# zfkuang/PaletteNeRF

Hardware: AMD Instinct MI355X
Metric: rendered_samples_per_sec (higher is better)
Workload: dtype f32 (field: f16x3 split products, fp32 accumulate); 1 GPU; configs[1]: NeRF-synthetic lego geometry (scene S0), -m nerf inference, 800x800, 1 view(s)/step, camera moving (one pose of the path per step); march_mode=native, fused_field=True, field_precision=f16x3, half_tables=False, ray_order=tile8, frames_in_flight=1, gathered_floats_per_ray=0, rccl_ranks=1, parallelism=single GPU

## Files before the change

palettenerf_amd/csrc/frame.hip:

```cpp
#include "pnr_common.hpp"
#include "march_core.hpp"
#include "grid_core.hpp"
#include "field_core.hpp"
#include "frame_plan.hpp"
#include <hip/hip_ext.h>
#include <vector>
#include <stdlib.h>

uint64_t pnr_internal_edit_device_bytes();
int pnr_internal_edit_upload(const pnr_palette_edit* edit, void* dst, hipStream_t s);
int pnr_internal_palette_field_forward(const pnr_palette_field_args* a, pnr_stream_t stream, int waves12);

namespace pnr {

struct FrameCtl {
    int32_t n_alive, n_step, step, done;
    int32_t iterations, pad0;
    unsigned long long rendered;
    unsigned long long rows;
    int32_t pad1[6];
};
static_assert(sizeof(FrameCtl) == 64, "FrameCtl layout");

constexpr uint32_t kHdr = 4;
// ... 113 lines not shown
        if (fin.depth_raw) fin.depth_raw[r] = d;
        depth[r] = (fin.on & 2) ? finish_depth(fin, d, r) : d;
    }
    if (q < 3) { const float v = simage[(size_t)i * 3 + q]; image[(size_t)r * 3 + q] = (fin.on & 1) ? finish_channel(fin, v, sws[i], r, q) : v; }
    if (saux) {
        if (q * 4 < aux_stride) {
            float4 v = *reinterpret_cast<const float4*>(saux + (size_t)i * aux_stride + q * 4);
            if (q == 0 && (fin.on & 4)) {
                const float w = sws[i];
                v.x = finish_channel(fin, v.x, w, r, 0); v.y = finish_channel(fin, v.y, w, r, 1); v.z = finish_channel(fin, v.z, w, r, 2);
            }
            *reinterpret_cast<float4*>(aux + (size_t)r * aux_stride + q * 4) = v;
        }
    } else if (aux && (fin.on & 4) && q < 3) {
        aux[(size_t)r * aux_stride + q] = finish_channel(fin, aux[(size_t)r * aux_stride + q], sws[i], r, q);
    }
}

#ifdef PNR_MARCH_STATS
__device__ unsigned long long g_march_stats[8];
__device__ unsigned int g_march_max[64];
__device__ unsigned int g_march_hist[2][32];
__device__ unsigned int g_march_kinds[64][8];
#endif
__device__ __forceinline__ uint32_t shfl_xor_fresh(uint32_t v, int off) {
    int lane = (int)__builtin_amdgcn_mbcnt_hi(~0u, __builtin_amdgcn_mbcnt_lo(~0u, 0u));
    asm volatile("" : "+v"(lane));
    return (uint32_t)__builtin_amdgcn_ds_bpermute((lane ^ off) << 2, (int)v);
}
__device__ __forceinline__ unsigned long long shfl_xor_fresh(unsigned long long v, int off) {
    return ((unsigned long long)shfl_xor_fresh((uint32_t)(v >> 32), off) << 32) | shfl_xor_fresh((uint32_t)v, off);
}
__device__ __forceinline__ unsigned long long block_sum_u64(unsigned long long v, unsigned long long* sh ) {
    for (int off = PNR_WAVE / 2; off > 0; off >>= 1) v += shfl_xor_fresh(v, off);
    __syncthreads();
    if ((threadIdx.x & (PNR_WAVE - 1)) == 0) sh[threadIdx.x / PNR_WAVE] = v;
    __syncthreads();
    unsigned long long t = 0;
    for (int wv = 0; wv < (int)(kRayBlock / PNR_WAVE); wv++) t += sh[wv];
    return t;
}


#ifdef PNR_MARCH_TIMING
constexpr int kTimingWaves = 8192;
__device__ unsigned long long g_march_timing[kTimingWaves * 8];
__device__ int g_march_timing_iter = 3;
#define PNR_STAMP(k) do { if (timing && (threadIdx.x & 63) == 0) g_march_timing[(size_t)twave * 8 + (k)] = wall_clock64(); } while (0)
#else
#define PNR_STAMP(k) do { } while (0)
#endif
#ifndef PNR_MARCH_WAVES
#define PNR_MARCH_WAVES 4
#endif
#ifndef PNR_MARCH_WAVES_Q
#define PNR_MARCH_WAVES_Q 5
#endif
template <bool MIP, bool POW2, int MODE>
__global__ void __launch_bounds__(kRayBlock) __attribute__((amdgpu_waves_per_eu(MODE == 2 ? PNR_MARCH_WAVES_Q : PNR_MARCH_WAVES))) k_frame_march(const FrameCtl* __restrict__ prev, FrameCtl* __restrict__ cur, const int32_t* __restrict__ alive_prev,
                                                           int32_t* __restrict__ rays_alive, const int32_t* __restrict__ counts ,
                                                           int32_t* __restrict__ counts_cur ,
                                                           int32_t* __restrict__ scratch_rw, uint32_t N, uint32_t max_steps,
                                                           const int32_t* __restrict__ partials_prev, uint32_t n_partials_prev,
                                                           const float* __restrict__ rays_t, const float* __restrict__ rays_o,
                                                           const float* __restrict__ rays_d, MarchParams p, const uint8_t* __restrict__ grid,
                                                           const float* __restrict__ fars, float* __restrict__ xyzs, float* __restrict__ dirs,
                                                           float* __restrict__ deltas, const uint32_t* __restrict__ mip,
                                                           int32_t* __restrict__ emitted_partials , uint32_t budget,
                                                           int32_t* __restrict__ qctr_all , StragglerRec* __restrict__ qrecs,
                                                           uint8_t* __restrict__ rowflag ,
                                                           const float* __restrict__ noises ) {
    __shared__ int csum[kRayBlock / PNR_WAVE];
    __shared__ unsigned long long red[kRayBlock / PNR_WAVE];
    __shared__ CoopShared coop[MODE == 1 ? kRayBlock / PNR_WAVE : 1];
#ifdef PNR_MARCH_TIMING
    const bool timing = prev->iterations + 1 == g_march_timing_iter && blockIdx.x * (kRayBlock / PNR_WAVE) < (uint32_t)kTimingWaves;
    const uint32_t twave = blockIdx.x * (kRayBlock / PNR_WAVE) + threadIdx.x / PNR_WAVE;
#endif
    PNR_STAMP(0);
    constexpr int kCountLoads = 8, kMipLoads = 5;
    const uint32_t max_chunks = (N + kRayBlock - 1) / kRayBlock;
    int32_t cv[kCountLoads];
#pragma unroll
    for (int u = 0; u < kCountLoads; u++) {
        const uint32_t j = threadIdx.x + (uint32_t)u * kRayBlock;
        cv[u] = j < max_chunks ? counts[j] : 0;
    }
    const uint32_t slot0 = blockIdx.x * kRayBlock + threadIdx.x;
    int index0 = slot0 < N ? alive_prev[slot0] : -1;
    extern __shared__ uint32_t mip_smem[];
    const uint32_t mip_n = MIP ? 2 * p.mip_words + 8 : 0;
    const bool mip_fast = MIP && mip_n <= (uint32_t)kMipLoads * kRayBlock * 4 && (mip_n & 3u) == 0;
    if (mip_fast) {
#pragma unroll
        for (int u = 0; u < kMipLoads; u++) {
            const uint32_t i = (threadIdx.x + (uint32_t)u * kRayBlock) * 4;
            if (i < mip_n) __builtin_amdgcn_global_load_lds((const __attribute__((address_space(1))) void*)(&mip[i]),
                                                            (__attribute__((address_space(3))) void*)(&mip_smem[i]), 16, 0, 0);
        }
    }
    if (prev->done) { if (blockIdx.x == 0 && threadIdx.x == 0) *cur = *prev; asm volatile("s_waitcnt vmcnt(0)" ::: "memory"); return; }
    const uint32_t n_prev = (uint32_t)prev->n_alive, nchunks = (n_prev + kRayBlock - 1) / kRayBlock;
    if (blockIdx.x >= nchunks && blockIdx.x != 0) { if (threadIdx.x == 0) emitted_partials[blockIdx.x] = 0; asm volatile("s_waitcnt vmcnt(0)" ::: "memory"); return; }
    if (slot0 >= n_prev) index0 = -1;
    unsigned long long part = 0;
#pragma unroll
    for (int u = 0; u < kCountLoads; u++) {
        const uint32_t j = threadIdx.x + (uint32_t)u * kRayBlock;
        if (j >= nchunks) cv[u] = 0;
        part += ((unsigned long long)(uint32_t)cv[u] << 32) | (j < blockIdx.x ? (unsigned long long)(uint32_t)cv[u] : 0ull);
    }
    for (uint32_t j = threadIdx.x + kCountLoads * kRayBlock; j < nchunks; j += kRayBlock) {
        const unsigned long long v = (unsigned long long)(uint32_t)counts[j];
        part += (v << 32) | (j < blockIdx.x ? v : 0ull);
    }
    const unsigned long long sums = block_sum_u64(part, red);
    const uint32_t n_alive = (uint32_t)(sums >> 32);
    const uint32_t n_step = (uint32_t)schedule_n_step((int)N, (int)n_alive);
    const int step_now = prev->step + prev->n_step;
    const bool done = n_alive == 0 || (uint32_t)step_now >= max_steps;
    if (blockIdx.x == 0) {
        unsigned long long e = 0;
        for (uint32_t j = threadIdx.x; j < n_partials_prev; j += kRayBlock) e += (unsigned long long)partials_prev[j];
        const unsigned long long emitted_prev = block_sum_u64(e, red);
        if (threadIdx.x == 0) {
            FrameCtl c = *prev;
            c.rendered += emitted_prev;
            c.rows += (unsigned long long)n_prev * (unsigned long long)prev->n_step;
            c.step = step_now;
            c.iterations += 1;
            c.n_alive = (int32_t)n_alive;
            c.n_step = (int32_t)n_step;
            c.done = done;
            c.pad0 = scratch_rw[1];
            *cur = c;
            scratch_rw[2] = 0;
            qctr_all[((c.iterations + 1) & 1) * kQueueCtrs] = 0;
        }
    }
    if (done || blockIdx.x >= nchunks) { if (threadIdx.x == 0) emitted_partials[blockIdx.x] = 0; asm volatile("s_waitcnt vmcnt(0)" ::: "memory"); return; }
    const int lane = threadIdx.x & (PNR_WAVE - 1), wave = threadIdx.x / PNR_WAVE;
    PNR_STAMP(1);
    const uint32_t* mip_lds = nullptr;
    if (mip_fast) {
        asm volatile("s_waitcnt vmcnt(0)" ::: "memory");
        __syncthreads();
        mip_lds = mip_smem;
    } else {
        mip_lds = stage_mip(mip, MIP ? p.mip_words : 0);
    }
    PNR_STAMP(2);
    uint32_t emitted = 0;
    uint32_t base = (uint32_t)(sums & 0xffffffffull), summed_to = blockIdx.x;
    for (uint32_t chunk = blockIdx.x; chunk < nchunks; chunk += gridDim.x) {
        if (threadIdx.x == 0) counts_cur[chunk] = 0;
        int index = index0;
        if (chunk != blockIdx.x) {
            unsigned long long pre = 0;
            for (uint32_t j = summed_to + threadIdx.x; j < chunk; j += kRayBlock) pre += (unsigned long long)counts[j];
            base += (uint32_t)block_sum_u64(pre, red);
            summed_to = chunk;
            const uint32_t slot = chunk * kRayBlock + threadIdx.x;
            index = slot < n_prev ? alive_prev[slot] : -1;
        }
        const int keep = index >= 0 ? 1 : 0;
        const unsigned long long alive_mask = __ballot(keep);
        if (lane == 0) csum[wave] = __popcll(alive_mask);
        __syncthreads();
        int woff = 0;
        for (int wv = 0; wv < wave; wv++) woff += csum[wv];
        __syncthreads();
        PNR_STAMP(3);
        uint32_t n = 0, step = 0;
        float t = 0.0f, far = -FLT_MAX, last_t = 0.0f;
        RayCtx c = {};
        if (keep) {
            n = base + (uint32_t)woff + (uint32_t)__popcll(alive_mask & ((1ull << lane) - 1ull));
            rays_alive[n] = index;
            ctx_init(c, rays_o + (size_t)index * 3, rays_d + (size_t)index * 3, p, grid, mip_lds);
            t = rays_t[index];
            const BoxHit bh = clip_to_box(c, fars[index]);
            far = bh.far;
            const float noise = (noises && prev->iterations == -1) ? noises[index] : 0.0f;
            t = fmaf(clampf(t * c.dt_gamma, c.dt_min, c.dt_max), noise, t);
            last_t = t;
            t = skip_to_box<MIP && POW2>(c, bh, t);
        }
        PNR_STAMP(4);
#ifdef PNR_MARCH_TIMING
        uint32_t my_probes = 0;
#endif
#ifdef PNR_MARCH_STATS
        unsigned long long probes = 0, empties = 0;
        unsigned int kinds[8] = {0, 0, 0, 0, 0, 0, 0, 0};
#endif
        bool active = keep && t < far;
        [[maybe_unused]] bool queued = false;
        [[maybe_unused]] uint32_t step_queued = 0;
        for (uint32_t round = 0;; round++) {
            const unsigned long long am = __ballot(active);
            if (am == 0ull) break;
            if constexpr (MODE == 1) { if (p.coop && __popcll(am) <= kCoopRays) break; }
            if constexpr (MODE == 2) {
                const bool give_up = active && round - step >= budget;
                const unsigned long long gm = __ballot(give_up);
                if (gm != 0ull) {
                    int32_t* qctr = qctr_all + ((prev->iterations + 1) & 1) * kQueueCtrs;
                    const int leader = __ffsll((long long)gm) - 1;
                    int slot0 = 0;
                    if (lane == leader) slot0 = atomicAdd(&qctr[0], __popcll(gm));
                    slot0 = __builtin_amdgcn_readlane(slot0, leader);
                    if (give_up) {
                        StragglerRec r;
                        r.n = (int32_t)n; r.index = index; r.step = (int32_t)step; r.t = t; r.last_t = last_t; r.far = far; r.pad0 = 0; r.pad1 = 0;
                        qrecs[(uint32_t)slot0 + (uint32_t)__popcll(gm & ((1ull << lane) - 1ull))] = r;
                        queued = true; step_queued = step; active = false;
                    }
                    if (gm == am) break;
                }
            }
            if (active) {
                float x, y, z, dt;
#ifdef PNR_MARCH_TIMING
                my_probes++;
#endif
#ifdef PNR_MARCH_STATS
                probes++;
                int kind = 7;
                const bool hit = march_probe<MIP, POW2>(c, t, x, y, z, dt, &kind);
                kinds[kind & 7]++;
                if (!hit) empties++;
#else
                const bool hit = march_probe<MIP, POW2>(c, t, x, y, z, dt);
#endif
                if (hit) {
                    const size_t row = (size_t)n * n_step + step;
                    float* px = xyzs + row * 3;
                    float* pd = dirs + row * 3;
                    float* pl = deltas + row * 2;
                    px[0] = x; px[1] = y; px[2] = z;
                    pd[0] = c.dx; pd[1] = c.dy; pd[2] = c.dz;
                    t += dt;
                    pl[0] = dt; pl[1] = t - last_t;
                    last_t = t;
                    step++;
                }
                active = t < far && step < n_step;
            }
        }
        if constexpr (MODE == 1) {
            if (p.coop && __ballot(active) != 0ull)
                step = march_coop_tail<MIP, POW2>(coop[wave], p, grid, mip_lds, n_step, active, c, t, far, last_t, n, step, xyzs, dirs, deltas);
        }
#ifdef PNR_MARCH_STATS
        if (keep) {
            const int so = prev->iterations + 1 == 0 ? 0 : 4;
            if (atomicMax(&g_march_max[(prev->iterations + 1) & 63], (unsigned int)probes) < (unsigned int)probes)
                for (int kk = 0; kk < 8; kk++) g_march_kinds[(prev->iterations + 1) & 63][kk] = kinds[kk];
            atomicAdd(&g_march_stats[so + 0], probes); atomicAdd(&g_march_stats[so + 1], empties); atomicAdd(&g_march_stats[so + 3], 1ull);
            atomicAdd(&g_march_hist[so ? 1 : 0][probes > 31 ? 31 : (int)probes], 1u);
            for (int kk = 0; kk < 8; kk++) if (kinds[kk]) atomicAdd(&g_march_kinds[so ? 63 : 62][kk], kinds[kk]);
        }
        {
            unsigned long long mx = probes;
            for (int off = 32; off > 0; off >>= 1) { unsigned long long o = __shfl_xor(mx, off, 64); mx = o > mx ? o : mx; }
            if ((threadIdx.x & 63) == 0) atomicAdd(&g_march_stats[prev->iterations + 1 == 0 ? 2 : 6], mx);
        }
#endif
        if (keep) {
            emitted += step;
            if constexpr (MODE == 2) {
                uint8_t* pf = rowflag + (size_t)n * n_step;
                for (uint32_t k = 0; k < n_step; k++) pf[k] = (queued && k >= step_queued) ? 1 : 0;
                if (queued) step = n_step;
            }
            float* pl = deltas + ((size_t)n * n_step + step) * 2;
            for (; step < n_step; step++) { pl[0] = 0.0f; pl[1] = 0.0f; pl += 2; }
        }
        PNR_STAMP(5);
#ifdef PNR_MARCH_TIMING
        if (timing) {
            uint32_t mp = my_probes, ml = c.n_loads;
            for (int off = 32; off > 0; off >>= 1) { mp = max(mp, (uint32_t)__shfl_xor((int)mp, off, 64)); ml = max(ml, (uint32_t)__shfl_xor((int)ml, off, 64)); }
            const uint32_t crowd = (uint32_t)__popcll(__ballot(my_probes >= 5u));
            if ((threadIdx.x & 63) == 0) { g_march_timing[(size_t)twave * 8 + 6] = mp; g_march_timing[(size_t)twave * 8 + 7] = ml | ((unsigned long long)crowd << 16); }
        }
#endif
    }
    __shared__ uint32_t wsum[kRayBlock / PNR_WAVE];
    for (int off = PNR_WAVE / 2; off > 0; off >>= 1) emitted += shfl_xor_fresh(emitted, off);
    if ((threadIdx.x & (PNR_WAVE - 1)) == 0) wsum[threadIdx.x / PNR_WAVE] = emitted;
    __syncthreads();
    if (threadIdx.x == 0) {
        uint32_t tot = 0;
        for (int wv = 0; wv < (int)(kRayBlock / PNR_WAVE); wv++) tot += wsum[wv];
        emitted_partials[blockIdx.x] = (int32_t)tot;
    }
}

enum GridKind { GK_SINGLE = 0, GK_PAIR = 1, GK_TRIPLE = 2, GK_HALF1 = 3, GK_HALF2 = 4, GK_HALF3 = 5 };
struct GridArgs {
    const float* xyzs; const float* deltas;
    const void* table[3]; float* enc[3];
    const int32_t* offsets; LevelParams lp;
    uint32_t level_stride; float bound, two_bound, inv_two_bound ; uint32_t gridtype;
};
struct LevelCtx { uint32_t off0, hashmap_size, resolution; float scale; uint32_t kind; };
__device__ __forceinline__ LevelCtx level_ctx(const GridArgs& g, uint32_t level) {
    LevelCtx lc;
    lc.off0 = (uint32_t)g.offsets[level];
    lc.hashmap_size = (uint32_t)g.offsets[level + 1] - lc.off0;
    lc.scale = g.lp.scale[level];
    lc.resolution = g.lp.resolution[level];
    lc.kind = level_kind<3>(g.gridtype, lc.hashmap_size, lc.resolution);
    return lc;
}
template <uint32_t CMUL>
__device__ __forceinline__ bool grid_corner_rows(const GridArgs& g, const LevelCtx& lc, uint32_t b, uint32_t idxs[8], float pos[3]) {
    float xyz[3];
#pragma unroll
    for (int d = 0; d < 3; d++) xyz[d] = g.xyzs[(size_t)b * 3 + d];
    asm volatile("" : "+v"(xyz[0]), "+v"(xyz[1]), "+v"(xyz[2]));
    float in[3];
    if (!unit_cube_of(xyz, g.bound, g.two_bound, g.inv_two_bound, in)) return false;
    uint32_t pg[3];
    grid_cell<3>(in, lc.scale, false, pg, pos);
    corner_rows<3, CMUL>(lc.kind, g.gridtype, false, lc.hashmap_size, lc.resolution, pg, idxs);
    return true;
}
template <int KIND, bool ORDERED = true>
__device__ __forceinline__ void grid_row(const GridArgs& g, const LevelCtx& lc, uint32_t level, const void* __restrict__ table, float* __restrict__ enc0, uint32_t b) {
    uint32_t idxs[8];
    float pos[3];
    const size_t o = ((size_t)level * g.level_stride + b) * 2;
    if constexpr (KIND == GK_TRIPLE) {
        float4 out = make_float4(0.0f, 0.0f, 0.0f, 0.0f);
        float2 outc = make_float2(0.0f, 0.0f);
        if (grid_corner_rows<1>(g, lc, b, idxs, pos)) {
            f32x4 v[8];
            f32x2 vc[8];
            float ws[8];
            const f32x4* tab = static_cast<const f32x4*>(table) + (size_t)lc.off0 * 2;
#pragma unroll
            for (int i = 0; i < 8; i++) v[i] = tab[(size_t)idxs[i] * 2];
#pragma unroll
            for (int i = 0; i < 8; i++) vc[i] = reinterpret_cast<const f32x2*>(tab + 1)[(size_t)idxs[i] * 4];
            corner_weights<3>(pos, ws);
#pragma unroll
            for (uint32_t idx = 0; idx < 8; idx++) {
                out.x = fmaf(ws[idx], v[idx].x, out.x); out.y = fmaf(ws[idx], v[idx].y, out.y);
                out.z = fmaf(ws[idx], v[idx].z, out.z); out.w = fmaf(ws[idx], v[idx].w, out.w);
                outc.x = fmaf(ws[idx], vc[idx].x, outc.x); outc.y = fmaf(ws[idx], vc[idx].y, outc.y);
            }
        }
        *reinterpret_cast<float2*>(enc0 + o) = make_float2(out.x, out.y);
        *reinterpret_cast<float2*>(g.enc[1] + o) = make_float2(out.z, out.w);
        *reinterpret_cast<float2*>(g.enc[2] + o) = outc;
    } else {
        constexpr bool HALF = KIND == GK_HALF1 || KIND == GK_HALF2 || KIND == GK_HALF3;
        constexpr int NT = KIND == GK_HALF3 ? 3 : ((KIND == GK_HALF2 || KIND == GK_PAIR) ? 2 : 1);
        constexpr int NW = HALF ? (NT == 3 ? 4 : NT) : 2 * NT;
        typedef uint32_t RowT __attribute__((ext_vector_type(NW)));
        typedef typename std::conditional<HALF, __half, float>::type AccT;
        AccT out[HALF ? 2 * NW : NW];
#pragma unroll
        for (int ch = 0; ch < 2 * NT; ch++) out[ch] = AccT(0.0f);
        if (grid_corner_rows<1>(g, lc, b, idxs, pos)) cell_interp<RowT, HALF, ORDERED>(static_cast<const RowT*>(table) + lc.off0, idxs, pos, out);
        *reinterpret_cast<float2*>(enc0 + o) = make_float2(to_f32(out[0]), to_f32(out[1]));
        if constexpr (NT >= 2) *reinterpret_cast<float2*>(g.enc[1] + o) = make_float2(to_f32(out[2]), to_f32(out[3]));
        if constexpr (NT == 3) *reinterpret_cast<float2*>(g.enc[2] + o) = make_float2(to_f32(out[4]), to_f32(out[5]));
    }
}

__device__ __forceinline__ uint32_t dpp_swap_pair(uint32_t x) { return (uint32_t)__builtin_amdgcn_update_dpp(0, (int)x, 0xB1 , 0xF, 0xF, true); }
template <int KIND>
__device__ __forceinline__ void grid_pair_level(const GridArgs& g, const LevelCtx& lc, uint32_t level, const void* __restrict__ table, float* __restrict__ enc0, uint32_t b,
                                                const float (&in)[3], bool live, bool ok, bool odd, bool okA, bool okB) {
    static_assert(KIND == GK_SINGLE, "the one-table fp32 layout");
    constexpr int NW = 2;
    typedef f32x2 RowT;
    float pos[3];
    uint32_t pg[3], ag[3], bg[3];
    grid_cell<3>(in, lc.scale, false, pg, pos);
#pragma unroll
    for (int d = 0; d < 3; d++) {
        const uint32_t qg = dpp_swap_pair(pg[d]);
        ag[d] = odd ? qg : pg[d];
        bg[d] = odd ? pg[d] : qg;
    }
    uint32_t idxs[8];
    x_side_rows<1>(lc.kind, g.gridtype, lc.hashmap_size, lc.resolution, ag, odd ? 1u : 0u, idxs);
    x_side_rows<1>(lc.kind, g.gridtype, lc.hashmap_size, lc.resolution, bg, odd ? 1u : 0u, idxs + 4);
    const RowT* tab = static_cast<const RowT*>(table) + lc.off0;
    const RowT* p[8];
#pragma unroll
    for (int i = 0; i < 8; i++) p[i] = tab + idxs[i];
    RowT v[8] = {};
    if (okA && okB) load8_fresh(p, v);
    else if (okA) {
#pragma unroll
        for (int i = 0; i < 4; i++) v[i] = *(typename GlobalPtr<RowT>::type)(uintptr_t)p[i];
    } else {
#pragma unroll
        for (int i = 4; i < 8; i++) v[i] = *(typename GlobalPtr<RowT>::type)(uintptr_t)p[i];
    }
    float ws[8];
    corner_weights<3>(pos, ws);
    RowT cw[8];
#pragma unroll
    for (int jk = 0; jk < 4; jk++) {
        uint32_t wa[NW], wb[NW];
        __builtin_memcpy(wa, &v[jk], sizeof(wa));
        __builtin_memcpy(wb, &v[4 + jk], sizeof(wb));
#pragma unroll
        for (int w = 0; w < NW; w++) {
            const uint32_t sa = dpp_swap_pair(wa[w]), sb = dpp_swap_pair(wb[w]);
            cw[2 * jk][w] = __builtin_bit_cast(float, odd ? sb : wa[w]);
            cw[2 * jk + 1][w] = __builtin_bit_cast(float, odd ? wb[w] : sa);
        }
    }
    const size_t o = ((size_t)level * g.level_stride + b) * 2;
    float acc[NW];
    cell_chain<RowT, false>(cw, ws, acc);
    const float2 out = make_float2(acc[0], acc[1]);
    if (ok) *reinterpret_cast<float2*>(enc0 + o) = out;
    else if (live) *reinterpret_cast<float2*>(enc0 + o) = make_float2(0.0f, 0.0f);
}
template <int KIND>
__device__ __forceinline__ void grid_row_at(const GridArgs& g, const LevelCtx& lc, uint32_t level, const void* __restrict__ table, float* __restrict__ enc0, uint32_t b,
                                            const float (&in)[3]) {
    static_assert(KIND == GK_SINGLE, "the one-table fp32 layout");
    float pos[3], acc[2];
    uint32_t pg[3], idxs[8];
    grid_cell<3>(in, lc.scale, false, pg, pos);
    corner_rows<3, 1>(lc.kind, g.gridtype, false, lc.hashmap_size, lc.resolution, pg, idxs);
    cell_interp<f32x2, false, true>(static_cast<const f32x2*>(table) + lc.off0, idxs, pos, acc);
    *reinterpret_cast<float2*>(enc0 + ((size_t)level * g.level_stride + b) * 2) = make_float2(acc[0], acc[1]);
}
template <int KIND, uint32_t NLV>
__device__ __forceinline__ void grid_pair_rows(const GridArgs& g, const LevelCtx (&lcs)[NLV], const uint32_t (&levels)[NLV], const void* __restrict__ table, float* __restrict__ enc0,
// ... 599 lines not shown
static int32_t* counts_of(const FramePlan& p, int parity) { return p.w.scratch + kHdr + (uint32_t)(parity & 1) * (p.N / kRayBlock + 2); }

static void launch_last(const FramePlan& p, const FrameCtl* done_ctl) {
    FrameFinish fin = p.fin;
    fin.ctl = done_ctl;
    const bool sorted = p.ray_order != nullptr, aux = p.aux_stride != 0;
    if (!sorted && !fin.on && !fin.depth_raw) return;
    UnsortKernel kernel;
    uint32_t blocks;
    if (sorted && aux && p.aux_stride > 64) { kernel = k_frame_unsort_outputs<32>; blocks = cdiv(p.N, kRayBlock / 32); }
    else if (sorted && aux) { kernel = k_frame_unsort_outputs<16>; blocks = cdiv(p.N * 16, kRayBlock); }
    else { kernel = k_frame_unsort_outputs<4>; blocks = cdiv(p.N * 4, kRayBlock); }
    hipLaunchKernelGGL(kernel, dim3(blocks), dim3(kRayBlock), 0, as_stream(p.stream), p.N, p.ray_order, p.out_ws, p.out_depth, p.out_image,
                       sorted ? (const float*)p.out_aux : (const float*)nullptr, p.aux_stride, p.ray_ws, p.ray_depth, p.ray_image, p.ray_aux, fin);
}

static MarchKernel frame_march_kernel(bool mip, bool pow2, int mode) {
    if (mode == 2) return k_frame_march<true, true, 2>;
    if (mip && pow2) return k_frame_march<true, true, 1>;
    if (mip) return k_frame_march<true, false, 1>;
    return pow2 ? k_frame_march<false, true, 1> : k_frame_march<false, false, 1>;
}
static FieldKernel frame_field_kernel(int precision, int watch_overflow) {
    if (precision == PNR_FIELD_FP32) return k_frame_field<0, false>;
    if (precision == PNR_FIELD_F16X2) return watch_overflow ? k_frame_field<2, true> : k_frame_field<2, false>;
    return watch_overflow ? k_frame_field<1, true> : k_frame_field<1, false>;
}

static int make_frame_plan(const pnr_nerf_frame_args* a, const pnr_palette_frame_args* pal, pnr_stream_t stream, const FrameOpts& opt, FramePlan* plan) {
    if (!a) return PNR_ERR_INVALID;
    plan->N = a->N;
    if (a->N == 0) return PNR_OK;
    if (!a->rays_o || !a->rays_d || !a->nears || !a->fars || !a->bitfield || !a->embeddings || !a->offsets || !a->packed_weights || !a->weights_sum ||
        !a->depth || !a->image || !a->workspace)
        return PNR_ERR_INVALID;
    if (a->C == 0 || a->C > 16 || a->H == 0 || a->max_steps == 0 || a->num_levels != 16) return PNR_ERR_UNSUPPORTED;
    if (a->field_precision != PNR_FIELD_FP32 && a->field_precision != PNR_FIELD_F16X3 && a->field_precision != PNR_FIELD_F16X2) return PNR_ERR_UNSUPPORTED;
    FramePlan& p = *plan;
    p = FramePlan{};
    p.stream = stream; p.workspace = a->workspace; p.N = a->N; p.max_steps = a->max_steps; p.T_thresh = a->T_thresh; p.density_scale = a->density_scale; p.opt = opt;
    p.aux_stride = pal ? pnr_palette_aux_channels(pal->num_basis, pal->clip_dim) : 0;
    p.with_clip = pal && pal->pred_clip;
    const FrameWorkspace& w = p.w = carve(a->workspace, p.N, p.aux_stride, p.with_clip);
    if (a->workspace_bytes < w.bytes) return PNR_ERR_INVALID;
    FrameCtl*& host_ctl = frame_device().host_ctl;
    if (!host_ctl && hipHostMalloc(reinterpret_cast<void**>(&host_ctl), sizeof(FrameCtl), hipHostMallocPortable) != hipSuccess) return PNR_ERR_LAUNCH;

    p.ray_order = a->ray_order;
    p.ray_ws = a->weights_sum; p.ray_depth = a->depth; p.ray_image = a->image; p.ray_aux = pal ? pal->aux_map : nullptr;
    const bool sorted = a->ray_order != nullptr;
    p.in_o = sorted ? w.s_o : a->rays_o; p.in_d = sorted ? w.s_d : a->rays_d; p.in_far = sorted ? w.s_far : a->fars;
    p.out_ws = sorted ? w.s_ws : p.ray_ws; p.out_depth = sorted ? w.s_depth : p.ray_depth; p.out_image = sorted ? w.s_image : p.ray_image;
    p.out_aux = sorted ? w.s_aux : p.ray_aux;
    p.noise_p = a->noises ? (sorted ? w.s_noise : a->noises) : nullptr;
    p.bitfield = a->bitfield; p.mip = static_cast<const uint32_t*>(a->mip); p.packed_weights = a->packed_weights;
    p.stats = a->stats; p.kernel_ms = a->kernel_ms; p.timing = a->kernel_ms != nullptr;

    p.n_enc = pal ? (p.with_clip ? 3u : 2u) : 1u;
    p.aux_fused = (pal && opt.aux_fusion && pnr_palette_field_stages_aux(pal->num_basis, pal->clip_dim, pal->pred_clip)) ? 1 : 0;
    p.composite_fused = (!pal && opt.composite_fusion) ? opt.composite_fusion : 0;
    p.pal_composite_fused = pal && p.aux_fused && opt.composite_fusion == 2;
    p.half_tables = a->table_dtype == PNR_DTYPE_F16;
    if (p.half_tables && pal && (p.with_clip ? !pal->embeddings_triple : !pal->embeddings_pair)) return PNR_ERR_UNSUPPORTED;
    if (a->table_dtype != PNR_DTYPE_F32 && a->table_dtype != PNR_DTYPE_F16) return PNR_ERR_UNSUPPORTED;

    GridArgs& ga = p.ga;
    ga.xyzs = w.xyzs; ga.deltas = w.deltas; ga.offsets = a->offsets; ga.lp = make_level_params(16, a->S, a->base_resolution); ga.level_stride = p.N;
    ga.bound = a->bound; ga.two_bound = 2.0f * a->bound; ga.inv_two_bound = exact_reciprocal_or_zero(ga.two_bound);
    ga.gridtype = a->gridtype;
    ga.enc[0] = w.enc; ga.enc[1] = w.enc_pal; ga.enc[2] = w.enc_clip;
    p.lookup_y = 16; p.lookup_z = 1;
    if (p.half_tables && pal && p.with_clip) { p.lookup = k_frame_grid_h3; ga.table[0] = pal->embeddings_triple; }
    else if (p.half_tables && pal) { p.lookup = k_frame_grid_h2; ga.table[0] = pal->embeddings_pair; }
    else if (p.half_tables) { p.lookup = k_frame_grid_h1; ga.table[0] = a->embeddings; }
    else if (pal && p.with_clip && pal->embeddings_triple) { p.lookup = k_frame_grid_triple; ga.table[0] = pal->embeddings_triple; }
    else if (pal && !p.with_clip && pal->embeddings_pair) { p.lookup = k_frame_grid_pair; ga.table[0] = pal->embeddings_pair; p.lookup_y = 16; }
    else {
        p.lookup = opt.grid_lane_pairs ? k_frame_grid_lp : k_frame_grid; p.lookup_y = 8; p.lookup_z = p.n_enc;
        ga.table[0] = a->embeddings; ga.table[1] = pal ? pal->embeddings_palette : nullptr; ga.table[2] = p.with_clip ? pal->embeddings_clip : nullptr;
    }

    if (pal) {
        pnr_palette_field_args& pf = p.pf;
        pf.enc = w.enc; pf.enc_palette = w.enc_pal; pf.enc_clip = w.enc_clip; pf.level_stride = p.N; pf.dirs = w.dirs; pf.deltas = w.deltas;
        pf.packed = a->packed_weights; pf.num_basis = pal->num_basis;
        pf.clip_dim = pal->clip_dim; pf.pred_clip = pal->pred_clip; pf.density_scale = a->density_scale; pf.offsets_weight = pal->offsets_weight;
        pf.view_dep_weight = pal->view_dep_weight; pf.aux_stride = p.aux_stride; pf.sigmas = w.sigmas; pf.rgbs = w.rgbs; pf.aux = w.aux;
        pf.precision = a->field_precision; pf.xyzs = w.xyzs;
        for (int k = 0; k < 3; k++) pf.enc_scale[k] = a->enc_scale[k];
        pf.overflow_flag = a->watch_overflow ? w.scratch + 1 : nullptr;
        pf.tile_counter = opt.dynamic_tiles ? w.scratch + 2 : nullptr;
        if (p.aux_fused) { pf.weights_sum = p.out_ws; pf.aux_map = p.out_aux; pf.T_thresh = a->T_thresh; }
        if (p.pal_composite_fused) { pf.rays_t = w.rays_t; pf.weights_sum_rw = p.out_ws; pf.depth = p.out_depth; pf.image = p.out_image; }
        if (pal->edit && pal->edit->mode != 0) { p.has_edit = true; p.edit = *pal->edit; pf.edit_device = w.edit; }
    } else {
        p.enc_scale = a->enc_scale[0] > 0.0f ? a->enc_scale[0] : 1.0f;
        p.field = frame_field_kernel(a->field_precision, a->watch_overflow);
    }

    p.use_mip = a->mip && (a->H % 4) == 0 && pnr_occupancy_mip_bytes(a->C, a->H) <= 64 * 1024;
    p.pow2 = is_pow2f(a->bound) && (a->H & (a->H - 1)) == 0;
    p.mp = make_march_params(a->bound, a->dt_gamma, a->max_steps, a->C, a->H, p.use_mip);
    p.mp.block_skip = opt.block_skip ? 1u : 0u; p.mp.coop = opt.coop_march ? 1u : 0u;
    p.march_lds = p.mp.mip_words ? (2 * p.mp.mip_words + 8) * 4 : 0;
    p.hosted = opt.hosted_tail && p.use_mip && p.pow2 && p.mp.mip_words != 0 && (a->H % 64u) == 0;
    p.march = frame_march_kernel(p.use_mip, p.pow2, 1); p.march_budgeted = frame_march_kernel(true, true, 2);

    FrameFinish& fin = p.fin;
    fin.on = a->finish; fin.bg[0] = a->bg_color[0]; fin.bg[1] = a->bg_color[1]; fin.bg[2] = a->bg_color[2];
    fin.bg_map = a->bg_map; fin.nears = a->nears; fin.fars = a->fars;
    fin.depth_raw = a->depth_raw;
    return PNR_OK;
}

static int frame_begin(const pnr_nerf_frame_args* a, const FramePlan& p) {
    const FrameWorkspace& w = p.w;
    hipStream_t s = as_stream(p.stream);
    if (p.has_edit) {
        const int rc = pnr_internal_edit_upload(&p.edit, w.edit, s);
        if (rc != PNR_OK) return rc;
    }
    HostedConst hconst = {};
    hconst.qctr_all = w.qctr; hconst.qrecs = w.qrecs; hconst.rays_o = p.in_o; hconst.rays_d = p.in_d; hconst.bitfield = p.bitfield; hconst.mip = p.mip; hconst.p = p.mp;
    hconst.xyzs = w.xyzs; hconst.dirs = w.dirs; hconst.deltas = w.deltas; hconst.partials[0] = w.partials[0]; hconst.partials[1] = w.partials[1];
    FrameBegin fb = {};
    fb.order = a->ray_order; fb.rays_o = a->rays_o; fb.rays_d = a->rays_d; fb.nears_in = a->nears; fb.fars_in = a->fars;
    fb.aabb = a->aabb; fb.min_near = a->min_near; fb.nears_out = a->nears; fb.fars_out = a->fars;
    fb.so = w.s_o; fb.sd = w.s_d; fb.sf = w.s_far; fb.noises = a->noises; fb.snoise = w.s_noise;
    if (p.aux_stride) {
        if ((p.aux_stride & 3u) == 0 && (reinterpret_cast<uintptr_t>(p.out_aux) & 15u) == 0) { fb.aux_zero = p.out_aux; fb.aux_stride = p.aux_stride; }
        else if (hipMemsetAsync(p.out_aux, 0, (size_t)p.N * p.aux_stride * 4, s) != hipSuccess) return PNR_ERR_LAUNCH;
    }
    hipLaunchKernelGGL(k_frame_begin, dim3(cdiv(p.N, kRayBlock)), dim3(kRayBlock), 0, s, p.N, fb, w.alive[1], w.rays_t, p.out_ws, p.out_depth, p.out_image,
                       w.ctl, counts_of(p, 1), w.scratch, w.qctr, hconst, w.hosted);
    return PNR_OK;
}

static hipEvent_t next_event(PerDevice& dev, FrameProgress& g) {
    if (g.ev_used == dev.ev.size()) { hipEvent_t e; if (hipEventCreate(&e) != hipSuccess) return nullptr; dev.ev.push_back(e); }
    return dev.ev[g.ev_used++];
}

static int enqueue_iteration(const FramePlan& p, FrameProgress& g, PerDevice& dev, bool look) {
    const FrameWorkspace& w = p.w;
    hipStream_t s = as_stream(p.stream);
    const int iter = g.iter;
    FrameCtl* cur = w.ctl + (iter & 1);
    const FrameCtl* prev = w.ctl + ((iter + 1) & 1);
    int32_t* alive_in = w.alive[iter & 1];
    const int32_t* alive_prev = w.alive[(iter + 1) & 1];
    const uint32_t rows_ub = rows_upper_bound(g.alive_ub, p.N);
    const uint32_t budget = march_budget(p.hosted, iter, p.opt.march_budget0, p.opt.march_budget);
    const int mode = march_mode(budget);
    const dim3 gm(march_blocks(g.alive_ub, mode, p.opt.march_blocks)), bm(kRayBlock);
    hipLaunchKernelGGL(mode == 2 ? p.march_budgeted : p.march, gm, bm, p.march_lds, s, prev, cur, alive_prev, alive_in, counts_of(p, iter + 1), counts_of(p, iter),
                       w.scratch, p.N, p.max_steps, w.partials[(iter + 1) & 1], g.prev_partials, w.rays_t, p.in_o, p.in_d, p.mp, p.bitfield, p.in_far, w.xyzs, w.dirs,
                       w.deltas, p.mip, w.partials[iter & 1], budget, w.qctr, w.qrecs, w.rowflag, p.noise_p);
    if (look) {
        if (hipMemcpyAsync(dev.host_ctl, cur, sizeof(FrameCtl), hipMemcpyDeviceToHost, s) != hipSuccess) return PNR_ERR_LAUNCH;
        if (!dev.done_ev && hipEventCreateWithFlags(&dev.done_ev, hipEventDisableTiming) != hipSuccess) return PNR_ERR_LAUNCH;
        if (hipEventRecord(dev.done_ev, s) != hipSuccess) return PNR_ERR_LAUNCH;
    }
    const uint32_t gxc = lookup_blocks_capped(rows_ub);
    HostedArgs ha = {};
    if (mode == 2) { ha.hc = w.hosted; ha.rowflag = w.rowflag; ha.blocks = kHostedBlocks; ha.partial_base = gm.x; ha.gx = gxc; ha.n_tab = p.n_enc; }
    hipEvent_t e0 = p.timing ? next_event(dev, g) : nullptr, e1 = p.timing ? next_event(dev, g) : nullptr;
    hipExtLaunchKernelGGL(p.lookup, ha.blocks ? dim3(ha.blocks + gxc * p.lookup_y * p.lookup_z) : dim3(gxc, p.lookup_y, p.lookup_z), dim3(256),
                          mode == 2 ? p.march_lds : 0u, s, e0, e1, 0, cur, p.ga, ha);
    if (p.aux_stride) {
        pnr_palette_field_args pf = p.pf;
        pf.ctl = cur; pf.B = rows_ub; pf.edit = p.has_edit ? &p.edit : nullptr;
        if (p.aux_fused) pf.rays_alive = alive_in;
        if (p.pal_composite_fused) { pf.rays_alive_rw = alive_in; pf.counts_cur = counts_of(p, iter); }
        const int rc = pnr_internal_palette_field_forward(&pf, p.stream, p.opt.palette_waves12);
        if (rc != PNR_OK) return rc;
    } else
        hipLaunchKernelGGL(p.field, dim3(field_blocks(rows_ub)), dim3(kFieldThreads), 0, s, cur, w.enc, p.N, w.dirs, w.deltas, p.packed_weights, p.density_scale,
                           p.enc_scale, w.sigmas, w.rgbs, p.composite_fused, p.T_thresh, alive_in, w.rays_t, p.out_ws, p.out_depth, p.out_image, w.scratch,
                           counts_of(p, iter));
    if (p.composite_fused != 2 && !p.pal_composite_fused)
        hipLaunchKernelGGL(k_frame_composite, gm, bm, 0, s, cur, p.T_thresh, alive_in, w.rays_t, w.sigmas, w.rgbs, w.deltas, p.out_ws, p.out_depth, p.out_image,
                           counts_of(p, iter), (const float*)w.aux, p.out_aux, p.aux_stride, p.aux_fused, p.composite_fused);
    g.prev_partials = gm.x + ha.blocks;
    return PNR_OK;
}

static int enqueue_chunk(const FramePlan& p, FrameProgress& g, PerDevice& dev) {
    for (uint32_t k = 0; k < g.chunk; k++, g.iter++)
        if (int rc = enqueue_iteration(p, g, dev, k + 1 == g.chunk)) return rc;
    launch_last(p, p.w.ctl + ((g.iter - 1) & 1));
    return PNR_OK;
}

static int frame_wait(const FramePlan& p, FrameProgress& g, PerDevice& dev) {
    const FrameCtl* host_ctl = dev.host_ctl;
    for (;;) {
        if (hipEventSynchronize(dev.done_ev) != hipSuccess) return PNR_ERR_LAUNCH;
        if (host_ctl->done) break;
        g.alive_ub = (uint32_t)host_ctl->n_alive;
        g.chunk = next_chunk(g.chunk, g.looks, dev.predicted_iterations);
        if (int rc = enqueue_chunk(p, g, dev)) return rc;
    }
    dev.predicted_iterations = (uint32_t)host_ctl->iterations;
    if (p.timing) {
        float total = 0.0f;
        uint32_t counted = 0;
        for (size_t i = 0; i + 1 < g.ev_used && counted < (uint32_t)host_ctl->iterations; i += 2, counted++) {
            float ms = 0.0f;
            if (hipEventElapsedTime(&ms, dev.ev[i], dev.ev[i + 1]) == hipSuccess) total += ms;
        }
        p.kernel_ms[0] = total;
        p.kernel_ms[1] = (float)counted * (float)p.lookup_z;
    }
    if (p.stats) {
        p.stats[0] = (uint64_t)host_ctl->iterations;
        p.stats[1] = host_ctl->rendered;
        p.stats[2] = host_ctl->rows;
        p.stats[3] = (uint64_t)g.iter;
        p.stats[4] = (uint64_t)g.looks + 1;
        p.stats[5] = (uint64_t)(host_ctl->pad0 != 0);
    }
    return check_launch();
}

enum FramePhase { kWhole = 0, kSubmit = 1, kFinish = 2 };
static int render_frame_impl(const void* args, const pnr_nerf_frame_args* a, const pnr_palette_frame_args* pal, pnr_stream_t stream, FramePhase phase) {
    if (phase == kFinish) {
        if (!a) return PNR_ERR_INVALID;
        if (a->N == 0) return PNR_OK;
        PerDevice& dev = frame_device();
        PerDevice::Pending& pending = dev.pending;
        if (!pending.on || pending.args != args) return PNR_ERR_INVALID;
        if (pending.plan.stream != stream || pending.plan.N != a->N || pending.plan.workspace != a->workspace) return PNR_ERR_INVALID;
        pending.on = false;
        return frame_wait(pending.plan, pending.prog, dev);
    }
    FramePlan plan;
    const int rc = make_frame_plan(a, pal, stream, frame_opts_now(), &plan);
    if (rc != PNR_OK || plan.N == 0) return rc;
    PerDevice& dev = frame_device();
    if (dev.pending.on && phase == kSubmit) return PNR_ERR_INVALID;
    dev.pending.on = false;
    FrameProgress prog;
    prog.alive_ub = plan.N;
    prog.chunk = first_chunk(dev.predicted_iterations, (uint32_t)plan.opt.iteration_margin);
    if (int rc2 = frame_begin(a, plan)) return rc2;
    if (int rc2 = enqueue_chunk(plan, prog, dev)) return rc2;
    if (phase == kWhole) return frame_wait(plan, prog, dev);
    dev.pending.args = args; dev.pending.plan = plan; dev.pending.prog = prog; dev.pending.on = true;
    return check_launch();
}

}

using namespace pnr;

extern "C" {

int pnr_interleave_tables(const float* a, const float* b, uint64_t rows, float* out, pnr_stream_t stream) {
    if (rows == 0) return PNR_OK;
    if (!a || !b || !out) return PNR_ERR_INVALID;
    hipLaunchKernelGGL(k_interleave_tables, dim3((uint32_t)((rows + 255) / 256)), dim3(256), 0, as_stream(stream), reinterpret_cast<const float2*>(a),
                       reinterpret_cast<const float2*>(b), rows, reinterpret_cast<float4*>(out));
    return check_launch();
}

int pnr_interleave_tables3(const float* a, const float* b, const float* c, uint64_t rows, float* out, pnr_stream_t stream) {
    if (rows == 0) return PNR_OK;
    if (!a || !b || !c || !out) return PNR_ERR_INVALID;
    hipLaunchKernelGGL(k_interleave_tables3, dim3((uint32_t)((rows + 255) / 256)), dim3(256), 0, as_stream(stream), reinterpret_cast<const float2*>(a),
                       reinterpret_cast<const float2*>(b), reinterpret_cast<const float2*>(c), rows, reinterpret_cast<float4*>(out));
    return check_launch();
}

int pnr_interleave_tables3_half(const float* a, const float* b, const float* c, uint64_t rows, void* out, pnr_stream_t stream) {
    if (rows == 0) return PNR_OK;
    if (!a || !b || !c || !out) return PNR_ERR_INVALID;
    hipLaunchKernelGGL(k_interleave_tables3_half, dim3((uint32_t)((rows + 255) / 256)), dim3(256), 0, as_stream(stream), reinterpret_cast<const float2*>(a),
                       reinterpret_cast<const float2*>(b), reinterpret_cast<const float2*>(c), rows, static_cast<uint4*>(out));
    return check_launch();
}

uint64_t pnr_nerf_frame_workspace_bytes(uint32_t N) { return carve(nullptr, N).bytes; }
uint64_t pnr_palette_frame_workspace_bytes(uint32_t N, uint32_t num_basis, uint32_t clip_dim, int pred_clip) {
    return carve(nullptr, N, pnr_palette_aux_channels(num_basis, clip_dim), pred_clip != 0).bytes;
}

int pnr_nerf_render_frame(const pnr_nerf_frame_args* a, pnr_stream_t stream) { return render_frame_impl(a, a, nullptr, stream, kWhole); }
int pnr_nerf_render_frame_submit(const pnr_nerf_frame_args* a, pnr_stream_t stream) { return render_frame_impl(a, a, nullptr, stream, kSubmit); }
int pnr_nerf_render_frame_finish(const pnr_nerf_frame_args* a, pnr_stream_t stream) { return render_frame_impl(a, a, nullptr, stream, kFinish); }

static int palette_frame(const pnr_palette_frame_args* p, pnr_stream_t stream, FramePhase phase) {
    if (!p) return PNR_ERR_INVALID;
    if (phase != kFinish) {
        if (p->num_basis < 1 || p->num_basis > PNR_MAX_BASIS || p->clip_dim > PNR_MAX_CLIP) return PNR_ERR_UNSUPPORTED;
        if (p->edit && (p->edit->mode < 0 || p->edit->mode > 2)) return PNR_ERR_UNSUPPORTED;
        if (p->base.N && (!p->embeddings_palette || !p->aux_map || (p->pred_clip && !p->embeddings_clip))) return PNR_ERR_INVALID;
    }
    return render_frame_impl(p, &p->base, p, stream, phase);
}
int pnr_palette_render_frame(const pnr_palette_frame_args* p, pnr_stream_t stream) { return palette_frame(p, stream, kWhole); }
int pnr_palette_render_frame_submit(const pnr_palette_frame_args* p, pnr_stream_t stream) { return palette_frame(p, stream, kSubmit); }
int pnr_palette_render_frame_finish(const pnr_palette_frame_args* p, pnr_stream_t stream) { return palette_frame(p, stream, kFinish); }

}

#ifdef PNR_MARCH_TIMING
// ... 42 lines not shown
```

palettenerf_amd/csrc/frame_plan.hpp:

```cpp
#pragma once
#include <stdint.h>

namespace pnr {

constexpr uint32_t kRayBlock = 256;
#ifndef PNR_MAX_MARCH_BLOCKS
#define PNR_MAX_MARCH_BLOCKS 4096
#endif
constexpr uint32_t kMaxMarchBlocks = PNR_MAX_MARCH_BLOCKS;
constexpr uint32_t kResidentMarchBlocks = 1280;

inline uint64_t align256(uint64_t v) { return (v + 255) & ~uint64_t(255); }
inline uint32_t plan_cdiv(uint32_t a, uint32_t b) { return (a + b - 1) / b; }
inline uint32_t plan_min(uint32_t a, uint32_t b) { return a < b ? a : b; }

inline uint32_t first_chunk(uint32_t predicted, uint32_t margin) {
    return predicted ? plan_min(predicted + 1u + margin, 1024u) : 8u;
}
inline uint32_t next_chunk(uint32_t chunk, uint32_t& looks, uint32_t predicted) {
    if (looks == 0) chunk = predicted ? 4u : 8u;
    if (++looks >= 4 && chunk < 64) chunk *= 2;
    return chunk;
}
inline uint32_t rows_upper_bound(uint32_t alive_ub, uint32_t N) { return (uint64_t)alive_ub * 8 < N ? alive_ub * 8 : N; }
inline uint32_t lookup_blocks(uint32_t rows_ub) { return plan_cdiv(rows_ub, 256); }
inline uint32_t lookup_blocks_capped(uint32_t rows_ub) { return plan_min(lookup_blocks(rows_ub), 1024u); }
inline uint32_t field_blocks(uint32_t rows_ub) { return plan_min(lookup_blocks(rows_ub), 512u); }
constexpr uint32_t field_wave_tile(uint32_t it, uint32_t wave, uint32_t block, uint32_t grid, uint32_t waves) {
    return it * grid * waves + (wave / 4u) * (grid * 4u) + block * 4u + (wave % 4u);
}
inline uint32_t march_budget(bool hosted, int iter, int budget_first, int budget_later) { return hosted ? (uint32_t)(iter == 0 ? budget_first : budget_later) : 0u; }
inline int march_mode(uint32_t budget) { return budget ? 2 : 1; }
inline uint32_t march_blocks(uint32_t alive_ub, int mode, int march_blocks_option) {
    const uint32_t ray_blocks = plan_cdiv(alive_ub, kRayBlock);
    uint32_t cap = kMaxMarchBlocks;
    if (mode == 2) {
        if (march_blocks_option > 0 && march_blocks_option < 65536) cap = plan_min((uint32_t)march_blocks_option, kMaxMarchBlocks);
        else if (ray_blocks >= 2 * kResidentMarchBlocks) cap = kResidentMarchBlocks;
    }
    return plan_min(ray_blocks, cap);
}

}
```

Baseline: 3.211 billion samples/s.

## Process later march chunks per wave without block-wide barriers

Restructures the persistent march loop. The first chunk is still handled block-wide, but each later 64-ray run is handled by a single wave, which computes its prefix offset from counts with a wave-level reduction and from ballots over the earlier runs in its chunk. This removes the __syncthreads pairs and block-wide reductions on each extra chunk iteration, so waves can move ahead independently. In exchange, every wave reloads the earlier runs' alive indices and redundantly sums the counts prefix, and the chunk counter clearing now depends on run ordering.

```diff
diff --git a/palettenerf_amd/csrc/frame.hip b/palettenerf_amd/csrc/frame.hip
--- a/palettenerf_amd/csrc/frame.hip
+++ b/palettenerf_amd/csrc/frame.hip
@@ -289,30 +289,14 @@
     PNR_STAMP(2);
     uint32_t emitted = 0;
     uint32_t base = (uint32_t)(sums & 0xffffffffull), summed_to = blockIdx.x;
-    for (uint32_t chunk = blockIdx.x; chunk < nchunks; chunk += gridDim.x) {
-        if (threadIdx.x == 0) counts_cur[chunk] = 0;
-        int index = index0;
-        if (chunk != blockIdx.x) {
-            unsigned long long pre = 0;
-            for (uint32_t j = summed_to + threadIdx.x; j < chunk; j += kRayBlock) pre += (unsigned long long)counts[j];
-            base += (uint32_t)block_sum_u64(pre, red);
-            summed_to = chunk;
-            const uint32_t slot = chunk * kRayBlock + threadIdx.x;
-            index = slot < n_prev ? alive_prev[slot] : -1;
-        }
+    const auto march_slots = [&](const int index, const unsigned long long alive_mask, const uint32_t first) __attribute__((always_inline)) {
         const int keep = index >= 0 ? 1 : 0;
-        const unsigned long long alive_mask = __ballot(keep);
-        if (lane == 0) csum[wave] = __popcll(alive_mask);
-        __syncthreads();
-        int woff = 0;
-        for (int wv = 0; wv < wave; wv++) woff += csum[wv];
-        __syncthreads();
         PNR_STAMP(3);
         uint32_t n = 0, step = 0;
         float t = 0.0f, far = -FLT_MAX, last_t = 0.0f;
         RayCtx c = {};
         if (keep) {
-            n = base + (uint32_t)woff + (uint32_t)__popcll(alive_mask & ((1ull << lane) - 1ull));
+            n = first + (uint32_t)__popcll(alive_mask & ((1ull << lane) - 1ull));
             rays_alive[n] = index;
             ctx_init(c, rays_o + (size_t)index * 3, rays_d + (size_t)index * 3, p, grid, mip_lds);
             t = rays_t[index];
@@ -423,6 +407,39 @@
             if ((threadIdx.x & 63) == 0) { g_march_timing[(size_t)twave * 8 + 6] = mp; g_march_timing[(size_t)twave * 8 + 7] = ml | ((unsigned long long)crowd << 16); }
         }
 #endif
+    };
+    {
+        if (threadIdx.x == 0) counts_cur[blockIdx.x] = 0;
+        const unsigned long long alive_mask = __ballot(index0 >= 0);
+        if (lane == 0) csum[wave] = __popcll(alive_mask);
+        __syncthreads();
+        int woff = 0;
+        for (int wv = 0; wv < wave; wv++) woff += csum[wv];
+        __syncthreads();
+        march_slots(index0, alive_mask, base + (uint32_t)woff);
+    }
+    const uint32_t nruns = march_runs(n_prev), wave_u = (uint32_t)__builtin_amdgcn_readfirstlane(wave);
+    for (uint32_t it = 1;; it++) {
+        const uint32_t run = march_run(it, wave_u, blockIdx.x, gridDim.x);
+        if (run >= nruns) break;
+        const uint32_t chunk = march_run_chunk(run);
+        const uint32_t slot = run * kRunRays + (uint32_t)lane;
+        const int index = slot < n_prev ? alive_prev[slot] : -1;
+        int earlier[kChunkRuns - 1];
+#pragma unroll
+        for (uint32_t u = 0; u + 1 < kChunkRuns; u++) {
+            const uint32_t s = (chunk * kChunkRuns + u) * kRunRays + (uint32_t)lane;
+            earlier[u] = (u < wave_u && s < n_prev) ? alive_prev[s] : -1;
+        }
+        uint32_t pre = march_lane_presum(counts, summed_to, chunk, (uint32_t)lane);
+        for (int off = PNR_WAVE / 2; off > 0; off >>= 1) pre += shfl_xor_fresh(pre, off);
+        base += pre;
+        summed_to = chunk;
+        uint32_t woff = 0;
+#pragma unroll
+        for (uint32_t u = 0; u + 1 < kChunkRuns; u++) woff += (uint32_t)__popcll(__ballot(earlier[u] >= 0));
+        if (march_run_clears(run) && lane == 0) counts_cur[chunk] = 0;
+        march_slots(index, __ballot(index >= 0), base + woff);
     }
     __shared__ uint32_t wsum[kRayBlock / PNR_WAVE];
     for (int off = PNR_WAVE / 2; off > 0; off >>= 1) emitted += shfl_xor_fresh(emitted, off);
@@ -1328,7 +1345,7 @@
     const uint32_t rows_ub = rows_upper_bound(g.alive_ub, p.N);
     const uint32_t budget = march_budget(p.hosted, iter, p.opt.march_budget0, p.opt.march_budget);
     const int mode = march_mode(budget);
-    const dim3 gm(march_blocks(g.alive_ub, mode, p.opt.march_blocks)), bm(kRayBlock);
+    const dim3 gm(march_run_blocks(g.alive_ub, mode, p.opt.march_blocks)), bm(kRayBlock);
     hipLaunchKernelGGL(mode == 2 ? p.march_budgeted : p.march, gm, bm, p.march_lds, s, prev, cur, alive_prev, alive_in, counts_of(p, iter + 1), counts_of(p, iter),
                        w.scratch, p.N, p.max_steps, w.partials[(iter + 1) & 1], g.prev_partials, w.rays_t, p.in_o, p.in_d, p.mp, p.bitfield, p.in_far, w.xyzs, w.dirs,
                        w.deltas, p.mip, w.partials[iter & 1], budget, w.qctr, w.qrecs, w.rowflag, p.noise_p);
diff --git a/palettenerf_amd/csrc/frame_plan.hpp b/palettenerf_amd/csrc/frame_plan.hpp
--- a/palettenerf_amd/csrc/frame_plan.hpp
+++ b/palettenerf_amd/csrc/frame_plan.hpp
@@ -40,5 +40,26 @@
     }
     return plan_min(ray_blocks, cap);
 }
+constexpr uint32_t kRunRays = 64, kChunkRuns = kRayBlock / kRunRays;
+constexpr uint32_t march_run(uint32_t it, uint32_t wave, uint32_t block, uint32_t grid) { return (it * grid + block) * kChunkRuns + wave; }
+constexpr uint32_t march_run_chunk(uint32_t run) { return run / kChunkRuns; }
+constexpr uint32_t march_runs(uint32_t n_prev) { return n_prev / kRunRays + (n_prev % kRunRays ? 1u : 0u); }
+constexpr uint32_t kPresumLoads = kResidentMarchBlocks / kRunRays;
+constexpr uint32_t march_lane_presum(const int32_t* counts, uint32_t summed_to, uint32_t chunk, uint32_t lane) {
+    uint32_t pre = 0;
+    for (uint32_t j0 = summed_to + lane; j0 < chunk; j0 += kPresumLoads * kRunRays) {
+        int32_t v[kPresumLoads] = {};
+#pragma unroll
+        for (uint32_t u = 0; u < kPresumLoads; u++) {
+            const uint32_t j = j0 + u * kRunRays;
+            if (j < chunk) v[u] = counts[j];
+        }
+#pragma unroll
+        for (uint32_t u = 0; u < kPresumLoads; u++) pre += (uint32_t)v[u];
+    }
+    return pre;
+}
+constexpr bool march_run_clears(uint32_t run) { return run % kChunkRuns == 0; }
+inline uint32_t march_run_blocks(uint32_t alive_ub, int mode, int march_blocks_option) { return march_blocks(alive_ub, mode, march_blocks_option); }
 
 }
```

Measured after the change: 3.210 billion samples/s (median of 2 runs). About the same (-0.0%).
